# Boey-li/AdaptiGraph

Hardware: AMD Instinct MI355X
Metric: rollout graph-steps/s (batch x rollout steps / wall; edge build + GNN forward + state update per graph-step) (higher is better)
Workload: dtype f16+fp8corr+bf16x3; 1 GPU; rope 1000+tool particles, batch 256/GPU, 10-step rollout (BASELINE configs[1]); global_batch=256, rollout_steps=10, parallelism=batch-shard x1 + all-gather, rollout_streams=1, weights=seed-0 random init (reference default init), precision=fast, model_status=0, self_edges=1, agg_q16=1

## Files before the change

adaptigraph_amd/csrc/ag_node_update_ws.hip:

```cpp
#include "ag_mlp_dev.h"

namespace {

#define AG_NWS_SET 20480
struct NwsUnit { bf16x8 hi[10], lo[10]; };

template <bool ACC>
__device__ __forceinline__ void nws_load_unit(NwsUnit &W, const float4 *chunk, int lane)
{
#pragma unroll
    for (int u = 0; u < 10; ++u) {
        W.hi[u] = *reinterpret_cast<const bf16x8 *>(chunk + (2 * u) * 64 + lane);
        W.lo[u] = *reinterpret_cast<const bf16x8 *>(chunk + (2 * u + 1) * 64 + lane);
    }
#pragma unroll
    for (int u = 0; u < 10; ++u) {
        if constexpr (ACC) asm volatile("" : "+a"(W.hi[u]), "+a"(W.lo[u]));
        else asm volatile("" : "+v"(W.hi[u]), "+v"(W.lo[u]));
    }
}
template <bool ACC>
__device__ __forceinline__ void nws_mfma3(f32x16 &acc, const bf16x8 &wh, const bf16x8 &wl, const bf16x8 &xh, const bf16x8 &xl)
{
    if constexpr (ACC)
        asm volatile("s_nop 1\n\tv_mfma_f32_32x32x16_bf16 %0, %1, %3, %0\n\tv_mfma_f32_32x32x16_bf16 %0, %2, %4, %0\n\tv_mfma_f32_32x32x16_bf16 %0, %2, %3, %0"
                     : "+v"(acc) : "a"(wl), "a"(wh), "v"(xh), "v"(xl));
    else
        asm volatile("s_nop 1\n\tv_mfma_f32_32x32x16_bf16 %0, %1, %3, %0\n\tv_mfma_f32_32x32x16_bf16 %0, %2, %4, %0\n\tv_mfma_f32_32x32x16_bf16 %0, %2, %3, %0"
                     : "+v"(acc) : "v"(wl), "v"(wh), "v"(xh), "v"(xl));
}
__device__ __forceinline__ void nws_settle(f32x16 &a) { asm volatile("s_nop 15\n\ts_nop 7" : "+v"(a)); }
template <int NU, bool ACC0, bool ACC1, bool ACC2>
__device__ __forceinline__ void nws_layer(f32x16 (&acc)[NU], const NwsUnit &W0, const NwsUnit &W1, const NwsUnit &W2, unsigned la)
{
    bf16x8 xq[3][2];
    lds_read16<0>(xq[0][0], la);
    lds_read16<1024>(xq[0][1], la);
    lds_read16<2048>(xq[1][0], la);
    lds_read16<3072>(xq[1][1], la);
    static_for<0, 10>([&](auto UU) {
        constexpr int u = decltype(UU)::value;
        if constexpr (u + 2 < 10) {
            lds_read16<(2 * (u + 2)) * 1024>(xq[(u + 2) % 3][0], la);
            lds_read16<(2 * (u + 2) + 1) * 1024>(xq[(u + 2) % 3][1], la);
        }
        constexpr int ahead = (9 - u) < 2 ? (9 - u) : 2;
        lds_wait_pair<2 * ahead>(xq[u % 3][0], xq[u % 3][1]);
        nws_mfma3<ACC0>(acc[0], W0.hi[u], W0.lo[u], xq[u % 3][0], xq[u % 3][1]);
        if constexpr (NU >= 2) nws_mfma3<ACC1>(acc[1], W1.hi[u], W1.lo[u], xq[u % 3][0], xq[u % 3][1]);
        if constexpr (NU >= 3) nws_mfma3<ACC2>(acc[NU - 1], W2.hi[u], W2.lo[u], xq[u % 3][0], xq[u % 3][1]);
    });
#pragma unroll
    for (int k = 0; k < NU; ++k) nws_settle(acc[k]);
}
__device__ __forceinline__ void nws_write_half(unsigned char *set_lane, int step, const float (&x)[8])
{
    typedef unsigned u32x4 __attribute__((ext_vector_type(4)));
    u32x4 H, L;
#pragma unroll
    for (int w = 0; w < 4; ++w) {
        const unsigned hp = cvt_pk_bf16(x[2 * w], x[2 * w + 1]);
        const float h0 = __uint_as_float(hp << 16), h1 = __uint_as_float(hp & 0xffff0000u);
        H[w] = hp;
        L[w] = cvt_pk_bf16(x[2 * w] - h0, x[2 * w + 1] - h1);
    }
    *reinterpret_cast<u32x4 *>(set_lane + (2 * step) * 1024) = H;
    *reinterpret_cast<u32x4 *>(set_lane + (2 * step + 1) * 1024) = L;
}

template <int WAVE, bool HSQ, bool AQ>
__device__ __forceinline__ void nws_wave(const AgWeights &w, const AgFwdArgs &a, unsigned char *sX, unsigned char *sY)
{
    constexpr int N1 = WAVE == 3 ? 2 : 1, N2 = WAVE == 1 ? 2 : 1, N3 = WAVE == 2 ? 2 : 1;
    constexpr int N23 = N2 + N3;
    const int lane = threadIdx.x & 63, j = lane & 31, h = lane >> 5;
    const int Mn = ag_rows(a);
    const int nblk = (Mn + 31) / 32;
    const int n_i = ((int)blockIdx.x < nblk) ? (nblk - (int)blockIdx.x + (int)gridDim.x - 1) / (int)gridDim.x : 0;
    const bool ovf = a.ovf && *a.ovf != 0;
    const float *pn_rows = ovf ? nullptr : a.pn_rows, *h_rows = ovf ? nullptr : a.h_rows;
    NwsUnit U1[N1], U2[N2], U3[N3];
    const float4 *ws = w.node_mid_b3;
    nws_load_unit<true>(U1[0], ws + (size_t)(0 + WAVE) * AG_CHUNK_F4, lane);
    nws_load_unit<true>(U2[0], ws + (size_t)(5 + WAVE) * AG_CHUNK_F4, lane);
    nws_load_unit<true>(U3[0], ws + (size_t)(10 + WAVE) * AG_CHUNK_F4, lane);
    if constexpr (N1 == 2) nws_load_unit<false>(U1[1], ws + (size_t)(0 + 4) * AG_CHUNK_F4, lane);
    if constexpr (N2 == 2) nws_load_unit<false>(U2[1], ws + (size_t)(5 + 4) * AG_CHUNK_F4, lane);
    if constexpr (N3 == 2) nws_load_unit<false>(U3[1], ws + (size_t)(10 + 4) * AG_CHUNK_F4, lane);
    const int t1[2] = {WAVE, 4}, t2[2] = {WAVE, 4}, t3[2] = {WAVE, 4};
    auto gblock = [&](int i) { return (int)blockIdx.x + i * (int)gridDim.x; };
    constexpr int NS = WAVE < 2 ? 3 : 2;
    float4 raw[AQ ? 1 : NS][2];
    int4 rawq[AQ ? NS : 1];
    uint2 rawex;
    auto stage_load = [&](int i) {
        const size_t g0 = (size_t)(i < n_i ? gblock(i) : 0) * 32 + j;
        const size_t g = g0 < (size_t)Mn ? g0 : 0;
        if constexpr (AQ) {
            const unsigned char *rowb = reinterpret_cast<const unsigned char *>(a.agg) + g * (2 * AG_FP);
#pragma unroll
            for (int k = 0; k < NS; ++k) {
                const int u = WAVE + 4 * k;
                rawq[k] = *reinterpret_cast<const int4 *>(rowb + 64 * (u >> 1) + 32 * h + 16 * (u & 1));
            }
            rawex = *reinterpret_cast<const uint2 *>(rowb + 280);
        } else {
            const float *row = a.agg + g * AG_FP + 4 * h;
#pragma unroll
            for (int k = 0; k < NS; ++k) {
                const int u = WAVE + 4 * k;
                raw[k][0] = *reinterpret_cast<const float4 *>(row + 16 * u);
                raw[k][1] = *reinterpret_cast<const float4 *>(row + 16 * u + 8);
            }
        }
    };
    auto stage_write = [&](unsigned char *set) {
#pragma unroll
        for (int k = 0; k < NS; ++k) {
            if constexpr (AQ) {
                const int u = WAVE + 4 * k;
                float x[8];
                agg_q16_decode8(rawq[k], agg_q16_tile_scale(rawex, u >> 1), x);
                if (u == 9) {
                    if (h) { x[2] = 0.0f; x[3] = 0.0f; }
                    x[4] = 0.0f; x[5] = 0.0f; x[6] = 0.0f; x[7] = 0.0f;
                }
                nws_write_half(set + lane * 16, u, x);
            } else {
                const float x[8] = {raw[k][0].x, raw[k][0].y, raw[k][0].z, raw[k][0].w, raw[k][1].x, raw[k][1].y, raw[k][1].z, raw[k][1].w};
                nws_write_half(set + lane * 16, WAVE + 4 * k, x);
            }
        }
    };
    f32x16 rh[N1];
    const float *pn_ptr = nullptr;
    int idx_raw = 0;
    const int32_t *idx_tab = pn_rows ? a.node_row : a.row_ptr;
    size_t crow_cur = 0;
    auto idx_load = [&](int i) {
        const size_t g = (size_t)(i < n_i ? gblock(i) : 0) * 32 + j;
        idx_raw = idx_tab[g < (size_t)Mn ? g : 0];
    };
    auto resid_load = [&](int i) {
        const int blk = i < n_i ? gblock(i) : 0;
        const size_t pk = (size_t)blk * AG_PACK_BLOCK + h * 128 + j * 4;
        pn_ptr = pn_rows ? pn_rows + crow_cur : a.pn + pk;
#pragma unroll
        for (int k = 0; k < N1; ++k) ResidInit::load_tile<true>(h_rows ? h_rows + crow_cur : a.h + pk, h_rows != nullptr, t1[k], rh[k]);
    };
    f32x16 acc1[N1];
    auto resid_to_acc = [&]() {
#pragma unroll
        for (int k = 0; k < N1; ++k) {
            f32x16 rp;
            ResidInit::load_tile(pn_ptr, pn_rows != nullptr, t1[k], rp);
            ResidInit::zero_pad(pn_rows != nullptr, t1[k], rp);
            ResidInit::zero_pad(h_rows != nullptr, t1[k], rh[k]);
#pragma unroll
            for (int r = 0; r < 16; ++r) acc1[k][r] = rp[r] + rh[k][r];
        }
    };
    idx_load(0);
    crow_cur = (size_t)idx_raw * AG_FP + 4 * h;
    stage_load(0);
    resid_load(0);
    idx_load(1);
    stage_write(sX);
    resid_to_acc();
    crow_cur = (size_t)idx_raw * AG_FP + 4 * h;
    __syncthreads();
#pragma unroll 1
    for (int p = 0; p <= n_i; ++p) {
        unsigned char *X = sX + (p & 1) * AG_NWS_SET, *Xn = sX + ((p + 1) & 1) * AG_NWS_SET;
        unsigned char *Y = sY + (p & 1) * AG_NWS_SET, *Yp = sY + ((p + 1) & 1) * AG_NWS_SET;
        if (p + 1 < n_i) { stage_load(p + 1); resid_load(p + 1); idx_load(p + 2); }
        if (p < n_i) {
            const int blk = gblock(p);
            nws_layer<N1, true, false, false>(acc1, U1[0], U1[N1 - 1], U1[N1 - 1], lds_addr_of(X) + lane * 16);
            const PackStoreEpi store{a.h + (size_t)blk * AG_PACK_BLOCK + h * 128 + j * 4};
#pragma unroll
            for (int k = 0; k < N1; ++k) {
#pragma unroll
                for (int r = 0; r < 16; ++r) acc1[k][r] = relu1(acc1[k][r]);
                store(t1[k], acc1[k]);
#pragma unroll
                for (int sh = 0; sh < 2; ++sh) {
                    const float x[8] = {acc1[k][8 * sh], acc1[k][8 * sh + 1], acc1[k][8 * sh + 2], acc1[k][8 * sh + 3],
                                        acc1[k][8 * sh + 4], acc1[k][8 * sh + 5], acc1[k][8 * sh + 6], acc1[k][8 * sh + 7]};
                    nws_write_half(Y + lane * 16, 2 * t1[k] + sh, x);
                }
            }
        }
        f32x16 acc[N23];
        const size_t g = (size_t)gblock(p >= 1 ? p - 1 : 0) * 32 + j;
        if (p >= 1) {
#pragma unroll
            for (int k = 0; k < N23; ++k)
#pragma unroll
                for (int r = 0; r < 16; ++r) acc[k][r] = 0.0f;
            const unsigned la = lds_addr_of(Yp) + lane * 16;
            if constexpr (N2 == 2) nws_layer<3, true, false, true>(acc, U2[0], U2[1], U3[0], la);
            else if constexpr (N3 == 2) nws_layer<3, true, true, false>(acc, U2[0], U3[0], U3[1], la);
            else nws_layer<2, true, true, false>(acc, U2[0], U3[0], U3[0], la);
        }
        if (p + 1 < n_i) { stage_write(Xn); resid_to_acc(); crow_cur = (size_t)idx_raw * AG_FP + 4 * h; }
        if (p >= 1) {
            const RowStoreEpi sr{a.hr_out + g * AG_FP + 4 * h};
#pragma unroll
            for (int k = 0; k < N2; ++k) sr(t2[k], acc[k]);
            if constexpr (HSQ) {
                const RowStoreQ16Epi sq{reinterpret_cast<unsigned char *>(a.hs_out) + g * (2 * AG_FP), h, a.status};
#pragma unroll
                for (int k = 0; k < N3; ++k) sq(t3[k], acc[N2 + k]);
            } else {
                const RowStoreEpi ss{a.hs_out + g * AG_FP + 4 * h};
#pragma unroll
                for (int k = 0; k < N3; ++k) ss(t3[k], acc[N2 + k]);
            }
        }
        ws_round_barrier();
    }
}

template <bool HSQ, bool AQ>
__global__ __launch_bounds__(256, 1) void node_update_nws_kernel(AgWeights w, AgFwdArgs a)
{
    __shared__ __attribute__((aligned(16))) unsigned char sX[2 * AG_NWS_SET], sY[2 * AG_NWS_SET];
    const int wave = __builtin_amdgcn_readfirstlane(threadIdx.x >> 6);
    if (wave == 0) nws_wave<0, HSQ, AQ>(w, a, sX, sY);
    else if (wave == 1) nws_wave<1, HSQ, AQ>(w, a, sX, sY);
    else if (wave == 2) nws_wave<2, HSQ, AQ>(w, a, sX, sY);
    else nws_wave<3, HSQ, AQ>(w, a, sX, sY);
}

}

void ag_launch_node_update_ws(const AgWeights &w, const AgFwdArgs &a, const AgNodeUpdate &v, hipStream_t s)
{
    const int cus = a.max_blocks / AG_MLP_WG_PER_CU > 0 ? a.max_blocks / AG_MLP_WG_PER_CU : 1, nblk = (a.B * a.N + 31) / 32;
    const dim3 g2(nblk < cus ? nblk : cus);
    if (v.agg_q16 && v.hs_q16) hipLaunchKernelGGL((node_update_nws_kernel<true, true>), g2, dim3(256), 0, s, w, a);
    else if (v.hs_q16) hipLaunchKernelGGL((node_update_nws_kernel<true, false>), g2, dim3(256), 0, s, w, a);
    else hipLaunchKernelGGL((node_update_nws_kernel<false, false>), g2, dim3(256), 0, s, w, a);
}
```

Baseline: 159,600 graph-steps/s.

## Split node-update warp specialization into 8 waves with layer-1 and table waves

Restructures the node-update kernel from 4 waves, each doing part of layer 1 plus part of the output layers, to 8 waves. Three waves compute layer 1, and five waves each compute two output tiles. Residual init moves to the table waves and is passed through a new LDS buffer. Staging is done by one wave, MFMA phases raise wave priority, and weight hi halves are pinned in AGPRs. The aim is to give each wave less MFMA work and more overlap, at the cost of more LDS and barrier traffic and 512-thread blocks.

```diff
diff --git a/adaptigraph_amd/csrc/ag_node_update_ws.hip b/adaptigraph_amd/csrc/ag_node_update_ws.hip
--- a/adaptigraph_amd/csrc/ag_node_update_ws.hip
+++ b/adaptigraph_amd/csrc/ag_node_update_ws.hip
@@ -5,7 +5,7 @@
 #define AG_NWS_SET 20480
 struct NwsUnit { bf16x8 hi[10], lo[10]; };
 
-template <bool ACC>
+template <bool ACCL>
 __device__ __forceinline__ void nws_load_unit(NwsUnit &W, const float4 *chunk, int lane)
 {
 #pragma unroll
@@ -15,43 +15,47 @@
     }
 #pragma unroll
     for (int u = 0; u < 10; ++u) {
-        if constexpr (ACC) asm volatile("" : "+a"(W.hi[u]), "+a"(W.lo[u]));
-        else asm volatile("" : "+v"(W.hi[u]), "+v"(W.lo[u]));
-    }
-}
-template <bool ACC>
+        asm volatile("" : "+a"(W.hi[u]));
+        if constexpr (ACCL) asm volatile("" : "+a"(W.lo[u]));
+        else asm volatile("" : "+v"(W.lo[u]));
+    }
+}
+template <bool ACCL>
 __device__ __forceinline__ void nws_mfma3(f32x16 &acc, const bf16x8 &wh, const bf16x8 &wl, const bf16x8 &xh, const bf16x8 &xl)
 {
-    if constexpr (ACC)
+    if constexpr (ACCL)
         asm volatile("s_nop 1\n\tv_mfma_f32_32x32x16_bf16 %0, %1, %3, %0\n\tv_mfma_f32_32x32x16_bf16 %0, %2, %4, %0\n\tv_mfma_f32_32x32x16_bf16 %0, %2, %3, %0"
                      : "+v"(acc) : "a"(wl), "a"(wh), "v"(xh), "v"(xl));
     else
         asm volatile("s_nop 1\n\tv_mfma_f32_32x32x16_bf16 %0, %1, %3, %0\n\tv_mfma_f32_32x32x16_bf16 %0, %2, %4, %0\n\tv_mfma_f32_32x32x16_bf16 %0, %2, %3, %0"
-                     : "+v"(acc) : "v"(wl), "v"(wh), "v"(xh), "v"(xl));
+                     : "+v"(acc) : "v"(wl), "a"(wh), "v"(xh), "v"(xl));
 }
 __device__ __forceinline__ void nws_settle(f32x16 &a) { asm volatile("s_nop 15\n\ts_nop 7" : "+v"(a)); }
-template <int NU, bool ACC0, bool ACC1, bool ACC2>
-__device__ __forceinline__ void nws_layer(f32x16 (&acc)[NU], const NwsUnit &W0, const NwsUnit &W1, const NwsUnit &W2, unsigned la)
-{
-    bf16x8 xq[3][2];
-    lds_read16<0>(xq[0][0], la);
-    lds_read16<1024>(xq[0][1], la);
-    lds_read16<2048>(xq[1][0], la);
-    lds_read16<3072>(xq[1][1], la);
+template <int NU>
+__device__ __forceinline__ void nws_phase(f32x16 (&acc)[NU], const NwsUnit (&W)[NU], unsigned la)
+{
+    constexpr int AH = NU == 1 ? 2 : 1, NS = AH + 1;
+    bf16x8 xq[NS][2];
+    __builtin_amdgcn_s_setprio(3);
+    static_for<0, AH>([&](auto UU) {
+        constexpr int u = decltype(UU)::value;
+        lds_read16<(2 * u) * 1024>(xq[u][0], la);
+        lds_read16<(2 * u + 1) * 1024>(xq[u][1], la);
+    });
     static_for<0, 10>([&](auto UU) {
         constexpr int u = decltype(UU)::value;
-        if constexpr (u + 2 < 10) {
-            lds_read16<(2 * (u + 2)) * 1024>(xq[(u + 2) % 3][0], la);
-            lds_read16<(2 * (u + 2) + 1) * 1024>(xq[(u + 2) % 3][1], la);
-        }
-        constexpr int ahead = (9 - u) < 2 ? (9 - u) : 2;
-        lds_wait_pair<2 * ahead>(xq[u % 3][0], xq[u % 3][1]);
-        nws_mfma3<ACC0>(acc[0], W0.hi[u], W0.lo[u], xq[u % 3][0], xq[u % 3][1]);
-        if constexpr (NU >= 2) nws_mfma3<ACC1>(acc[1], W1.hi[u], W1.lo[u], xq[u % 3][0], xq[u % 3][1]);
-        if constexpr (NU >= 3) nws_mfma3<ACC2>(acc[NU - 1], W2.hi[u], W2.lo[u], xq[u % 3][0], xq[u % 3][1]);
+        if constexpr (u + AH < 10) {
+            lds_read16<(2 * (u + AH)) * 1024>(xq[(u + AH) % NS][0], la);
+            lds_read16<(2 * (u + AH) + 1) * 1024>(xq[(u + AH) % NS][1], la);
+        }
+        constexpr int ahead = (9 - u) < AH ? (9 - u) : AH;
+        lds_wait_pair<2 * ahead>(xq[u % NS][0], xq[u % NS][1]);
+        nws_mfma3<true>(acc[0], W[0].hi[u], W[0].lo[u], xq[u % NS][0], xq[u % NS][1]);
+        if constexpr (NU == 2) nws_mfma3<false>(acc[1], W[1].hi[u], W[1].lo[u], xq[u % NS][0], xq[u % NS][1]);
     });
 #pragma unroll
     for (int k = 0; k < NU; ++k) nws_settle(acc[k]);
+    __builtin_amdgcn_s_setprio(0);
 }
 __device__ __forceinline__ void nws_write_half(unsigned char *set_lane, int step, const float (&x)[8])
 {
@@ -68,57 +72,58 @@
     *reinterpret_cast<u32x4 *>(set_lane + (2 * step + 1) * 1024) = L;
 }
 
-template <int WAVE, bool HSQ, bool AQ>
-__device__ __forceinline__ void nws_wave(const AgWeights &w, const AgFwdArgs &a, unsigned char *sX, unsigned char *sY)
-{
-    constexpr int N1 = WAVE == 3 ? 2 : 1, N2 = WAVE == 1 ? 2 : 1, N3 = WAVE == 2 ? 2 : 1;
-    constexpr int N23 = N2 + N3;
-    const int lane = threadIdx.x & 63, j = lane & 31, h = lane >> 5;
-    const int Mn = ag_rows(a);
-    const int nblk = (Mn + 31) / 32;
-    const int n_i = ((int)blockIdx.x < nblk) ? (nblk - (int)blockIdx.x + (int)gridDim.x - 1) / (int)gridDim.x : 0;
-    const bool ovf = a.ovf && *a.ovf != 0;
-    const float *pn_rows = ovf ? nullptr : a.pn_rows, *h_rows = ovf ? nullptr : a.h_rows;
-    NwsUnit U1[N1], U2[N2], U3[N3];
-    const float4 *ws = w.node_mid_b3;
-    nws_load_unit<true>(U1[0], ws + (size_t)(0 + WAVE) * AG_CHUNK_F4, lane);
-    nws_load_unit<true>(U2[0], ws + (size_t)(5 + WAVE) * AG_CHUNK_F4, lane);
-    nws_load_unit<true>(U3[0], ws + (size_t)(10 + WAVE) * AG_CHUNK_F4, lane);
-    if constexpr (N1 == 2) nws_load_unit<false>(U1[1], ws + (size_t)(0 + 4) * AG_CHUNK_F4, lane);
-    if constexpr (N2 == 2) nws_load_unit<false>(U2[1], ws + (size_t)(5 + 4) * AG_CHUNK_F4, lane);
-    if constexpr (N3 == 2) nws_load_unit<false>(U3[1], ws + (size_t)(10 + 4) * AG_CHUNK_F4, lane);
-    const int t1[2] = {WAVE, 4}, t2[2] = {WAVE, 4}, t3[2] = {WAVE, 4};
-    auto gblock = [&](int i) { return (int)blockIdx.x + i * (int)gridDim.x; };
-    constexpr int NS = WAVE < 2 ? 3 : 2;
-    float4 raw[AQ ? 1 : NS][2];
-    int4 rawq[AQ ? NS : 1];
-    uint2 rawex;
-    auto stage_load = [&](int i) {
-        const size_t g0 = (size_t)(i < n_i ? gblock(i) : 0) * 32 + j;
+struct NwsGeom {
+    int lane, j, h, Mn, n_i;
+    __device__ __forceinline__ explicit NwsGeom(const AgFwdArgs &a)
+    {
+        lane = threadIdx.x & 63; j = lane & 31; h = lane >> 5;
+        Mn = ag_rows(a);
+        const int nblk = (Mn + 31) / 32;
+        n_i = ((int)blockIdx.x < nblk) ? (nblk - (int)blockIdx.x + (int)gridDim.x - 1) / (int)gridDim.x : 0;
+    }
+    __device__ __forceinline__ int gblock(int i) const { return (int)blockIdx.x + i * (int)gridDim.x; }
+};
+
+template <int T0, int NT, bool STAGE, bool AQ>
+__device__ __forceinline__ void nws_first_wave(const AgWeights &w, const AgFwdArgs &a, unsigned char *sX, unsigned char *sY, const unsigned char *sR)
+{
+    const NwsGeom G(a);
+    const int lane = G.lane, j = G.j, h = G.h, Mn = G.Mn, n_i = G.n_i;
+    NwsUnit U[NT];
+    nws_load_unit<true>(U[0], w.node_mid_b3 + (size_t)T0 * AG_CHUNK_F4, lane);
+    if constexpr (NT == 2) nws_load_unit<false>(U[1], w.node_mid_b3 + (size_t)(T0 + 1) * AG_CHUNK_F4, lane);
+    constexpr int NH = AQ ? 1 : 2, SPH = 10 / NH;
+    float4 raw[AQ || !STAGE ? 1 : SPH][2];
+    int4 rawq[AQ && STAGE ? SPH : 1];
+    uint2 rawex = make_uint2(0u, 0u);
+    auto stage_load = [&](int i, auto HH) {
+        constexpr int u0 = decltype(HH)::value * SPH;
+        const size_t g0 = (size_t)(i < n_i ? G.gblock(i) : 0) * 32 + j;
         const size_t g = g0 < (size_t)Mn ? g0 : 0;
         if constexpr (AQ) {
             const unsigned char *rowb = reinterpret_cast<const unsigned char *>(a.agg) + g * (2 * AG_FP);
 #pragma unroll
-            for (int k = 0; k < NS; ++k) {
-                const int u = WAVE + 4 * k;
+            for (int k = 0; k < SPH; ++k) {
+                const int u = u0 + k;
                 rawq[k] = *reinterpret_cast<const int4 *>(rowb + 64 * (u >> 1) + 32 * h + 16 * (u & 1));
             }
             rawex = *reinterpret_cast<const uint2 *>(rowb + 280);
         } else {
             const float *row = a.agg + g * AG_FP + 4 * h;
 #pragma unroll
-            for (int k = 0; k < NS; ++k) {
-                const int u = WAVE + 4 * k;
+            for (int k = 0; k < SPH; ++k) {
+                const int u = u0 + k;
                 raw[k][0] = *reinterpret_cast<const float4 *>(row + 16 * u);
                 raw[k][1] = *reinterpret_cast<const float4 *>(row + 16 * u + 8);
             }
         }
     };
-    auto stage_write = [&](unsigned char *set) {
-#pragma unroll
-        for (int k = 0; k < NS; ++k) {
+    auto stage_write = [&](unsigned char *set, auto HH) {
+        constexpr int u0 = decltype(HH)::value * SPH;
+#pragma unroll
+        for (int k = 0; k < SPH; ++k) {
+            const int u = u0 + k;
             if constexpr (AQ) {
-                const int u = WAVE + 4 * k;
                 float x[8];
                 agg_q16_decode8(rawq[k], agg_q16_tile_scale(rawex, u >> 1), x);
                 if (u == 9) {
@@ -128,109 +133,136 @@
                 nws_write_half(set + lane * 16, u, x);
             } else {
                 const float x[8] = {raw[k][0].x, raw[k][0].y, raw[k][0].z, raw[k][0].w, raw[k][1].x, raw[k][1].y, raw[k][1].z, raw[k][1].w};
-                nws_write_half(set + lane * 16, WAVE + 4 * k, x);
-            }
-        }
-    };
-    f32x16 rh[N1];
+                nws_write_half(set + lane * 16, u, x);
+            }
+        }
+    };
+    auto stage_block = [&](int i, unsigned char *set, bool loaded0) {
+        if (!loaded0) stage_load(i, std::integral_constant<int, 0>{});
+        stage_write(set, std::integral_constant<int, 0>{});
+        if constexpr (NH == 2) {
+            stage_load(i, std::integral_constant<int, 1>{});
+            stage_write(set, std::integral_constant<int, 1>{});
+        }
+    };
+    if constexpr (STAGE) stage_block(0, sX, false);
+    __syncthreads();
+#pragma unroll 1
+    for (int p = 0; p <= n_i; ++p) {
+        unsigned char *X = sX + (p & 1) * AG_NWS_SET, *Xn = sX + ((p + 1) & 1) * AG_NWS_SET, *Y = sY + (p & 1) * AG_NWS_SET;
+        const unsigned char *R = sR + (p & 1) * AG_NWS_SET;
+        if constexpr (STAGE) { if (p + 1 < n_i) stage_load(p + 1, std::integral_constant<int, 0>{}); }
+        if (p < n_i) {
+            f32x16 acc[NT];
+#pragma unroll
+            for (int k = 0; k < NT; ++k)
+#pragma unroll
+                for (int q = 0; q < 4; ++q) {
+                    const float4 v = *reinterpret_cast<const float4 *>(R + (((T0 + k) * 4 + q) * 64 + lane) * 16);
+                    acc[k][4 * q] = v.x; acc[k][4 * q + 1] = v.y; acc[k][4 * q + 2] = v.z; acc[k][4 * q + 3] = v.w;
+                }
+            nws_phase<NT>(acc, U, lds_addr_of(X) + lane * 16);
+            if constexpr (STAGE) { if (p + 1 < n_i) stage_block(p + 1, Xn, true); }
+            const PackStoreEpi store{a.h + (size_t)G.gblock(p) * AG_PACK_BLOCK + h * 128 + j * 4};
+#pragma unroll
+            for (int k = 0; k < NT; ++k) {
+#pragma unroll
+                for (int r = 0; r < 16; ++r) acc[k][r] = relu1(acc[k][r]);
+                store(T0 + k, acc[k]);
+#pragma unroll
+                for (int sh = 0; sh < 2; ++sh) {
+                    const float x[8] = {acc[k][8 * sh], acc[k][8 * sh + 1], acc[k][8 * sh + 2], acc[k][8 * sh + 3],
+                                        acc[k][8 * sh + 4], acc[k][8 * sh + 5], acc[k][8 * sh + 6], acc[k][8 * sh + 7]};
+                    nws_write_half(Y + lane * 16, 2 * (T0 + k) + sh, x);
+                }
+            }
+        }
+        ws_round_barrier();
+    }
+}
+
+template <int LA, int TA, int LB, int TB, int RT, bool HSQ>
+__device__ __forceinline__ void nws_table_wave(const AgWeights &w, const AgFwdArgs &a, const unsigned char *sY, unsigned char *sR)
+{
+    const NwsGeom G(a);
+    const int lane = G.lane, j = G.j, h = G.h, Mn = G.Mn, n_i = G.n_i;
+    const bool ovf = a.ovf && *a.ovf != 0;
+    const float *pn_rows = ovf ? nullptr : a.pn_rows, *h_rows = ovf ? nullptr : a.h_rows;
+    NwsUnit U[2];
+    nws_load_unit<true>(U[0], w.node_mid_b3 + (size_t)(5 * LA + TA) * AG_CHUNK_F4, lane);
+    nws_load_unit<false>(U[1], w.node_mid_b3 + (size_t)(5 * LB + TB) * AG_CHUNK_F4, lane);
+    f32x16 acc[2];
+#pragma unroll
+    for (int r = 0; r < 16; ++r) acc[0][r] = acc[1][r] = 0.0f;
+    auto store_one = [&](auto LL, auto TT, const f32x16 &v, size_t g) {
+        constexpr int L = decltype(LL)::value, T = decltype(TT)::value;
+        if constexpr (L == 1) RowStoreEpi{a.hr_out + g * AG_FP + 4 * h}(T, v);
+        else if constexpr (HSQ) RowStoreQ16Epi{reinterpret_cast<unsigned char *>(a.hs_out) + g * (2 * AG_FP), h, a.status}(T, v);
+        else RowStoreEpi{a.hs_out + g * AG_FP + 4 * h}(T, v);
+    };
+    auto store = [&](int i) {
+        const size_t g = (size_t)G.gblock(i) * 32 + j;
+        store_one(std::integral_constant<int, LA>{}, std::integral_constant<int, TA>{}, acc[0], g);
+        store_one(std::integral_constant<int, LB>{}, std::integral_constant<int, TB>{}, acc[1], g);
+    };
+    f32x16 rh;
     const float *pn_ptr = nullptr;
     int idx_raw = 0;
     const int32_t *idx_tab = pn_rows ? a.node_row : a.row_ptr;
-    size_t crow_cur = 0;
+    size_t crow = 0;
     auto idx_load = [&](int i) {
-        const size_t g = (size_t)(i < n_i ? gblock(i) : 0) * 32 + j;
+        const size_t g = (size_t)(i < n_i ? G.gblock(i) : 0) * 32 + j;
         idx_raw = idx_tab[g < (size_t)Mn ? g : 0];
     };
     auto resid_load = [&](int i) {
-        const int blk = i < n_i ? gblock(i) : 0;
-        const size_t pk = (size_t)blk * AG_PACK_BLOCK + h * 128 + j * 4;
-        pn_ptr = pn_rows ? pn_rows + crow_cur : a.pn + pk;
-#pragma unroll
-        for (int k = 0; k < N1; ++k) ResidInit::load_tile<true>(h_rows ? h_rows + crow_cur : a.h + pk, h_rows != nullptr, t1[k], rh[k]);
-    };
-    f32x16 acc1[N1];
-    auto resid_to_acc = [&]() {
-#pragma unroll
-        for (int k = 0; k < N1; ++k) {
-            f32x16 rp;
-            ResidInit::load_tile(pn_ptr, pn_rows != nullptr, t1[k], rp);
-            ResidInit::zero_pad(pn_rows != nullptr, t1[k], rp);
-            ResidInit::zero_pad(h_rows != nullptr, t1[k], rh[k]);
-#pragma unroll
-            for (int r = 0; r < 16; ++r) acc1[k][r] = rp[r] + rh[k][r];
-        }
+        const size_t pk = (size_t)(i < n_i ? G.gblock(i) : 0) * AG_PACK_BLOCK + h * 128 + j * 4;
+        pn_ptr = pn_rows ? pn_rows + crow : a.pn + pk;
+        ResidInit::load_tile<true>(h_rows ? h_rows + crow : a.h + pk, h_rows != nullptr, RT, rh);
+    };
+    auto resid_write = [&](unsigned char *R) {
+        f32x16 rp;
+        ResidInit::load_tile(pn_ptr, pn_rows != nullptr, RT, rp);
+        ResidInit::zero_pad(pn_rows != nullptr, RT, rp);
+        ResidInit::zero_pad(h_rows != nullptr, RT, rh);
+#pragma unroll
+        for (int q = 0; q < 4; ++q)
+            *reinterpret_cast<float4 *>(R + ((RT * 4 + q) * 64 + lane) * 16) =
+                make_float4(rp[4 * q] + rh[4 * q], rp[4 * q + 1] + rh[4 * q + 1], rp[4 * q + 2] + rh[4 * q + 2], rp[4 * q + 3] + rh[4 * q + 3]);
     };
     idx_load(0);
-    crow_cur = (size_t)idx_raw * AG_FP + 4 * h;
-    stage_load(0);
+    crow = (size_t)idx_raw * AG_FP + 4 * h;
     resid_load(0);
     idx_load(1);
-    stage_write(sX);
-    resid_to_acc();
-    crow_cur = (size_t)idx_raw * AG_FP + 4 * h;
+    resid_write(sR);
+    crow = (size_t)idx_raw * AG_FP + 4 * h;
     __syncthreads();
 #pragma unroll 1
     for (int p = 0; p <= n_i; ++p) {
-        unsigned char *X = sX + (p & 1) * AG_NWS_SET, *Xn = sX + ((p + 1) & 1) * AG_NWS_SET;
-        unsigned char *Y = sY + (p & 1) * AG_NWS_SET, *Yp = sY + ((p + 1) & 1) * AG_NWS_SET;
-        if (p + 1 < n_i) { stage_load(p + 1); resid_load(p + 1); idx_load(p + 2); }
-        if (p < n_i) {
-            const int blk = gblock(p);
-            nws_layer<N1, true, false, false>(acc1, U1[0], U1[N1 - 1], U1[N1 - 1], lds_addr_of(X) + lane * 16);
-            const PackStoreEpi store{a.h + (size_t)blk * AG_PACK_BLOCK + h * 128 + j * 4};
-#pragma unroll
-            for (int k = 0; k < N1; ++k) {
-#pragma unroll
-                for (int r = 0; r < 16; ++r) acc1[k][r] = relu1(acc1[k][r]);
-                store(t1[k], acc1[k]);
-#pragma unroll
-                for (int sh = 0; sh < 2; ++sh) {
-                    const float x[8] = {acc1[k][8 * sh], acc1[k][8 * sh + 1], acc1[k][8 * sh + 2], acc1[k][8 * sh + 3],
-                                        acc1[k][8 * sh + 4], acc1[k][8 * sh + 5], acc1[k][8 * sh + 6], acc1[k][8 * sh + 7]};
-                    nws_write_half(Y + lane * 16, 2 * t1[k] + sh, x);
-                }
-            }
-        }
-        f32x16 acc[N23];
-        const size_t g = (size_t)gblock(p >= 1 ? p - 1 : 0) * 32 + j;
+        if (p + 1 < n_i) { resid_load(p + 1); idx_load(p + 2); }
         if (p >= 1) {
 #pragma unroll
-            for (int k = 0; k < N23; ++k)
-#pragma unroll
-                for (int r = 0; r < 16; ++r) acc[k][r] = 0.0f;
-            const unsigned la = lds_addr_of(Yp) + lane * 16;
-            if constexpr (N2 == 2) nws_layer<3, true, false, true>(acc, U2[0], U2[1], U3[0], la);
-            else if constexpr (N3 == 2) nws_layer<3, true, true, false>(acc, U2[0], U3[0], U3[1], la);
-            else nws_layer<2, true, true, false>(acc, U2[0], U3[0], U3[0], la);
-        }
-        if (p + 1 < n_i) { stage_write(Xn); resid_to_acc(); crow_cur = (size_t)idx_raw * AG_FP + 4 * h; }
-        if (p >= 1) {
-            const RowStoreEpi sr{a.hr_out + g * AG_FP + 4 * h};
-#pragma unroll
-            for (int k = 0; k < N2; ++k) sr(t2[k], acc[k]);
-            if constexpr (HSQ) {
-                const RowStoreQ16Epi sq{reinterpret_cast<unsigned char *>(a.hs_out) + g * (2 * AG_FP), h, a.status};
-#pragma unroll
-                for (int k = 0; k < N3; ++k) sq(t3[k], acc[N2 + k]);
-            } else {
-                const RowStoreEpi ss{a.hs_out + g * AG_FP + 4 * h};
-#pragma unroll
-                for (int k = 0; k < N3; ++k) ss(t3[k], acc[N2 + k]);
-            }
-        }
+            for (int r = 0; r < 16; ++r) acc[0][r] = acc[1][r] = 0.0f;
+            nws_phase<2>(acc, U, lds_addr_of(sY + ((p + 1) & 1) * AG_NWS_SET) + lane * 16);
+        }
+        if (p + 1 < n_i) { resid_write(sR + ((p + 1) & 1) * AG_NWS_SET); crow = (size_t)idx_raw * AG_FP + 4 * h; }
+        if (p >= 1) store(p - 1);
         ws_round_barrier();
     }
 }
 
 template <bool HSQ, bool AQ>
-__global__ __launch_bounds__(256, 1) void node_update_nws_kernel(AgWeights w, AgFwdArgs a)
-{
-    __shared__ __attribute__((aligned(16))) unsigned char sX[2 * AG_NWS_SET], sY[2 * AG_NWS_SET];
+__global__ __launch_bounds__(512, 1) void node_update_nws_kernel(AgWeights w, AgFwdArgs a)
+{
+    __shared__ __attribute__((aligned(16))) unsigned char sX[2 * AG_NWS_SET], sY[2 * AG_NWS_SET], sR[2 * AG_NWS_SET];
     const int wave = __builtin_amdgcn_readfirstlane(threadIdx.x >> 6);
-    if (wave == 0) nws_wave<0, HSQ, AQ>(w, a, sX, sY);
-    else if (wave == 1) nws_wave<1, HSQ, AQ>(w, a, sX, sY);
-    else if (wave == 2) nws_wave<2, HSQ, AQ>(w, a, sX, sY);
-    else nws_wave<3, HSQ, AQ>(w, a, sX, sY);
+    if (wave == 0) nws_first_wave<0, 2, false, AQ>(w, a, sX, sY, sR);
+    else if (wave == 1) nws_first_wave<2, 2, false, AQ>(w, a, sX, sY, sR);
+    else if (wave == 2) nws_first_wave<4, 1, true, AQ>(w, a, sX, sY, sR);
+    else if (wave == 3) nws_table_wave<1, 2, 1, 3, 0, HSQ>(w, a, sY, sR);
+    else if (wave == 4) nws_table_wave<1, 0, 1, 1, 1, HSQ>(w, a, sY, sR);
+    else if (wave == 5) nws_table_wave<2, 0, 2, 1, 2, HSQ>(w, a, sY, sR);
+    else if (wave == 6) nws_table_wave<1, 4, 2, 4, 3, HSQ>(w, a, sY, sR);
+    else nws_table_wave<2, 2, 2, 3, 4, HSQ>(w, a, sY, sR);
 }
 
 }
@@ -239,7 +271,7 @@
 {
     const int cus = a.max_blocks / AG_MLP_WG_PER_CU > 0 ? a.max_blocks / AG_MLP_WG_PER_CU : 1, nblk = (a.B * a.N + 31) / 32;
     const dim3 g2(nblk < cus ? nblk : cus);
-    if (v.agg_q16 && v.hs_q16) hipLaunchKernelGGL((node_update_nws_kernel<true, true>), g2, dim3(256), 0, s, w, a);
-    else if (v.hs_q16) hipLaunchKernelGGL((node_update_nws_kernel<true, false>), g2, dim3(256), 0, s, w, a);
-    else hipLaunchKernelGGL((node_update_nws_kernel<false, false>), g2, dim3(256), 0, s, w, a);
-}
+    if (v.agg_q16 && v.hs_q16) hipLaunchKernelGGL((node_update_nws_kernel<true, true>), g2, dim3(512), 0, s, w, a);
+    else if (v.hs_q16) hipLaunchKernelGGL((node_update_nws_kernel<true, false>), g2, dim3(512), 0, s, w, a);
+    else hipLaunchKernelGGL((node_update_nws_kernel<false, false>), g2, dim3(512), 0, s, w, a);
+}
```

After: 158,900 graph-steps/s, median of 3. About the same (-0.4%).
